# halajun/VDO_SLAM

Measured on AMD Instinct MI355X. Metric: frames/sec (per-frame hot path, KITTI-0000-shaped 1242x375) + ms/LM-iter (batch factor graph), higher is better.
Workload: dtype f64 (LM, RANSAC) / u8,i32,f32 (front-end, tracking)

## Files before the change

include/vdo_slam_hip.h:

```cpp
#ifndef VDO_SLAM_HIP_H_
#define VDO_SLAM_HIP_H_
#include <stdint.h>

#ifdef __cplusplus
extern "C" {
#endif

typedef enum vdo_status {
  VDO_OK = 0,
  VDO_ERR_INVALID = -1,
  VDO_ERR_NO_DEVICE = -2,
  VDO_ERR_OOM = -3,
  VDO_ERR_UNSUPPORTED = -4,
  VDO_ERR_INTERNAL = -5
} vdo_status;

int vdo_version(void);
const char* vdo_last_error(void);

typedef struct vdo_ctx vdo_ctx;
int vdo_ctx_create(int device, void* hip_stream, vdo_ctx** out);
int vdo_ctx_destroy(vdo_ctx* ctx);
int vdo_ctx_synchronize(vdo_ctx* ctx);
int vdo_ctx_stream(vdo_ctx* ctx, void** hip_stream_out);
// ... 74 lines not shown
int vdo_rccl_comm_destroy(vdo_rccl_comm* comm);
int vdo_rccl_comm_stats(const vdo_rccl_comm* comm, int64_t* calls, int64_t* bytes);
int vdo_rccl_allreduce(vdo_rccl_comm* comm, double* device_buf, int64_t count, int op );
int vdo_ba_set_rccl(vdo_ba* ba, vdo_rccl_comm* comm );
int vdo_ba_partition(const vdo_ba_graph* g, int world, int32_t* owner_of_point );
typedef struct vdo_ba_plan vdo_ba_plan;
int vdo_ba_plan_create(const vdo_ba_graph* g, vdo_ba_plan** out);
int vdo_ba_plan_array(const vdo_ba_plan* p, const char* name, const void** data, int64_t* count, int32_t* elem_bytes);
int vdo_ba_plan_destroy(vdo_ba_plan* p);

typedef struct vdo_flow2_problem {
  int32_t n;
  const double* obs;
  const double* flow;
  const double* depth;
  double K[4];
  double Twl[16];
  double T0[16];
  double info_flow;
  double info_prior;
  double huber_delta;
  double chi2_gate;
  int32_t max_iterations;
  int32_t ref_quirks;
} vdo_flow2_problem;

typedef struct vdo_flow2_result {
  double T[16];
  int32_t n_inliers;
  int32_t iterations, trials, stop_reason;
  double initial_chi2, final_chi2, final_lambda;
} vdo_flow2_result;

typedef struct vdo_flow2_batch vdo_flow2_batch;
int vdo_flow2_batch_create(vdo_ctx* ctx, int n_problems, const vdo_flow2_problem* probs, vdo_flow2_batch** out);
int vdo_flow2_batch_reserve(vdo_ctx* ctx, int n_problems, const int32_t* capacity, vdo_flow2_batch** out);
int vdo_flow2_batch_set(vdo_flow2_batch* batch, int k, const vdo_flow2_problem* problem);
int vdo_flow2_batch_run(vdo_flow2_batch* batch);
int vdo_flow2_batch_fetch(vdo_flow2_batch* batch, vdo_flow2_result* results, double** flow_out, uint8_t** inlier_out);
int vdo_flow2_batch_destroy(vdo_flow2_batch* batch);
int vdo_flow2_optimize(vdo_ctx* ctx, const vdo_flow2_problem* p, vdo_flow2_result* result, double* flow_out, uint8_t* inlier_out);

typedef struct vdo_pose_problem {
  int32_t n;
  int32_t kind;
  const double* obs;
  const double* Xw;
  double K[4];
  double P[12];
  double T0[16];
  double huber_delta;
  double chi2_gate;
  int32_t max_iterations;
  int32_t pad;
} vdo_pose_problem;

typedef struct vdo_pose_batch vdo_pose_batch;
int vdo_pose_batch_create(vdo_ctx* ctx, int n_problems, const vdo_pose_problem* probs, vdo_pose_batch** out);
int vdo_pose_batch_run(vdo_pose_batch* batch);
int vdo_pose_batch_fetch(vdo_pose_batch* batch, vdo_flow2_result* results, uint8_t** inlier_out);
int vdo_pose_batch_destroy(vdo_pose_batch* batch);
int vdo_pose_optimize(vdo_ctx* ctx, const vdo_pose_problem* p, vdo_flow2_result* result, uint8_t* inlier_out);

typedef struct vdo_pnp_problem {
  int32_t n;
  const double* X;
  const double* uv;
  double K[4];
  int32_t max_iterations;
  double reproj_threshold;
  double confidence;
  int32_t refit;
} vdo_pnp_problem;
typedef struct vdo_pnp_result {
  double T[16];
  int32_t n_inliers;
  int32_t iterations_run;
  int32_t best_iteration;
} vdo_pnp_result;
int vdo_pnp_ransac_batch(vdo_ctx* ctx, int n_problems, const vdo_pnp_problem* probs, vdo_pnp_result* results, uint8_t** inlier_out);
int vdo_pnp_ransac_batch_overlap(vdo_ctx* ctx, int n_problems, const vdo_pnp_problem* probs, vdo_pnp_result* results, uint8_t** inlier_out,
                                 void (*host_work)(void*), void* host_arg);
int vdo_pnp_ransac(vdo_ctx* ctx, const vdo_pnp_problem* p, vdo_pnp_result* result, uint8_t* inlier_out);

typedef struct vdo_orb_params {
  int32_t n_features;
  float scale_factor;
  int32_t n_levels;
  int32_t ini_th;
  int32_t min_th;
} vdo_orb_params;

typedef struct vdo_keypoints {
  int32_t capacity, n;
  float *x, *y, *response, *angle, *size;
  int32_t* octave;
} vdo_keypoints;

typedef struct vdo_orb vdo_orb;
int vdo_orb_create(vdo_ctx* ctx, const vdo_orb_params* prm, int width, int height, vdo_orb** out);
int vdo_orb_destroy(vdo_orb* orb);
int vdo_orb_max_keypoints(const vdo_orb* orb, int* n);
int vdo_orb_extract(vdo_orb* orb, const uint8_t* gray, int stride, int src_is_device, vdo_keypoints* out);
int vdo_orb_extract_begin(vdo_orb* orb, const uint8_t* gray, int stride, int src_is_device);
int vdo_orb_extract_end(vdo_orb* orb, vdo_keypoints* out);
int vdo_orb_descriptors(vdo_orb* orb, uint8_t* desc32, int capacity_rows);
int vdo_orb_extract_desc(vdo_orb* orb, const uint8_t* gray, int stride, int src_is_device, vdo_keypoints* out, uint8_t* desc32);
int vdo_orb_level_info(vdo_orb* orb, int level, int* w, int* h, int* n_features, int* n_candidates);
int vdo_orb_get_pyramid(vdo_orb* orb, int level, uint8_t* out_bordered );
int vdo_orb_get_blurred(vdo_orb* orb, int level, uint8_t* out );
int vdo_orb_get_candidates(vdo_orb* orb, int level, float* x, float* y, float* response, float* angle, int cap, int* n);
int vdo_orb_last_timing(vdo_orb* orb, double ms[2]);
int vdo_orb_pyramid_launches(const vdo_orb* orb);

int vdo_depth_preprocess(vdo_ctx* ctx, float* depth, int64_t n, float bf, float depth_map_factor, int is_device);
int vdo_rgb2gray(vdo_ctx* ctx, const uint8_t* rgb, int64_t n_pixels, int channels, int rgb_order, uint8_t* gray);

typedef struct vdo_frame_images vdo_frame_images;
int vdo_frame_images_create(vdo_ctx* ctx, int width, int height, vdo_frame_images** out);
int vdo_frame_images_upload(vdo_frame_images* f, const float* depth, const float* flow, const int32_t* mask);
int vdo_frame_images_upload_on(vdo_ctx* ctx, vdo_frame_images* f, const float* depth, const float* flow, const int32_t* mask);
int vdo_frame_images_upload_device(vdo_frame_images* f, const float* depth_dev, const float* flow_dev, const int32_t* mask_dev);
int vdo_frame_images_depth_preprocess(vdo_frame_images* f, float bf, float depth_map_factor);
int vdo_frame_images_ingest_device(vdo_frame_images* f, const float* depth_dev, const float* flow_dev, const int32_t* mask_dev, float bf, float depth_map_factor,
                                   int convert_depth);
int vdo_frame_images_destroy(vdo_frame_images* f);
int vdo_frame_images_set_ctx(vdo_frame_images* f, vdo_ctx* ctx);
int vdo_frame_static_filter(vdo_frame_images* f, int n, const float* kx, const float* ky, float th_depth,
                            int32_t* keep_idx, float* corr_x, float* corr_y, float* flow_x, float* flow_y,
                            float* depth_out, int* n_out);
int vdo_frame_static_filter_sampled(vdo_frame_images* f, int n, const float* kx, const float* ky, float th_depth,
                                    int32_t* keep_idx, float* corr_x, float* corr_y, float* flow_x, float* flow_y,
                                    float* depth_out, int* n_out);
int vdo_sample_keypoints(int rows, int cols, uint64_t seed, int capacity, float* x_out, float* y_out, int* n_out);
int vdo_frame_object_sample(vdo_frame_images* f, float th_depth_obj, int step, int cap,
                            float* key_x, float* key_y, float* corr_x, float* corr_y,
                            float* flow_x, float* flow_y, float* depth_out, int32_t* label, int* n_out);
int vdo_frame_object_sample_on(vdo_ctx* on_ctx, vdo_frame_images* f, float th_depth_obj, int step, int cap,
                               float* key_x, float* key_y, float* corr_x, float* corr_y,
                               float* flow_x, float* flow_y, float* depth_out, int32_t* label, int* n_out);
int vdo_frame_filters(vdo_frame_images* f, int n, const float* kx, const float* ky, float th_depth, int sampled,
                      int32_t* keep_idx, float* s_corr_x, float* s_corr_y, float* s_flow_x, float* s_flow_y, float* s_depth, int* n_static,
                      float th_depth_obj, int step, int cap,
                      float* key_x, float* key_y, float* corr_x, float* corr_y, float* flow_x, float* flow_y, float* depth_out, int32_t* label, int* n_obj);
int vdo_frame_filters_on(vdo_ctx* on_ctx, vdo_frame_images* f, int n, const float* kx, const float* ky, float th_depth, int sampled,
                         int32_t* keep_idx, float* s_corr_x, float* s_corr_y, float* s_flow_x, float* s_flow_y, float* s_depth, int* n_static,
                         float th_depth_obj, int step, int cap,
                         float* key_x, float* key_y, float* corr_x, float* corr_y, float* flow_x, float* flow_y, float* depth_out, int32_t* label, int* n_obj);


int vdo_propagate_static(vdo_frame_images* f, int n, const float* kx, const float* ky, float* depth_out);
int vdo_propagate_object(vdo_frame_images* f, int n, const float* kx, const float* ky, float th_depth_obj,
                         float* depth_out, int32_t* label_out);
int vdo_get3d_world(vdo_ctx* ctx, int n, const float* kx, const float* ky, const float* depth,
                    const float K4[4], const float Twc[16], float* xyz_out);
int vdo_scene_flow(vdo_ctx* ctx, int n, const float* cur_x, const float* cur_y, const float* cur_d, const int32_t* cur_label, const float Tcw_cur[16],
                   const float* last_x, const float* last_y, const float* last_d, const int32_t* last_label, const float Tcw_last[16],
                   const float K4[4], float* flow3d_out, int32_t* obj_label_inout);
int vdo_renew_static(vdo_frame_images* f, int n_tm, const int32_t* tm_sta, const float* stat_x, const float* stat_y,
                     int n_orb, const float* orb_x, const float* orb_y, int max_num_sta,
                     float* key_x, float* key_y, float* corr_x, float* corr_y, float* flow_x, float* flow_y,
                     int32_t* inlier_id, float* depth_out, int* n_out);
int vdo_renew_static_world(vdo_frame_images* f, int n_tm, const int32_t* tm_sta, const float* stat_x, const float* stat_y,
                           int n_orb, const float* orb_x, const float* orb_y, int max_num_sta, const float K4[4], const float Twc[16],
                           float* key_x, float* key_y, float* corr_x, float* corr_y, float* flow_x, float* flow_y,
                           int32_t* inlier_id, float* depth_out, float* xyz_out, int* n_out);
// ... 72 lines not shown
```

vdo_slam_amd/csrc/arena.hpp:

```cpp
#pragma once
#include <hip/hip_runtime.h>

#include <algorithm>
#include <cstdlib>
#include <cstring>
#include <vector>

#include "../../include/vdo_slam_hip.h"
#include "ctx.hpp"

namespace vdo {

class Arena {
 public:
  explicit Arena(vdo_ctx* c) : c_(c), s_(c->stream) {}
  hipStream_t stream() { flush(); return s_; }

  bool reserve(size_t bytes) {
    bytes = (bytes + 4095) & ~size_t(4095);
    if (bytes > c_->d_cap) {
      hipStreamSynchronize(s_);
      if (c_->d_arena) hipFree(c_->d_arena);
      c_->d_arena = nullptr; c_->d_cap = 0;
      const size_t want = bytes < (size_t(8) << 20) ? (size_t(8) << 20) : bytes * 2;
      if (hipMalloc((void**)&c_->d_arena, want) != hipSuccess) return false;
      c_->d_cap = want;
    }
    if (bytes > c_->h_cap) {
      hipStreamSynchronize(s_);
      if (c_->h_arena) hipHostFree(c_->h_arena);
      c_->h_arena = nullptr; c_->h_cap = 0; c_->h_arena_dev = nullptr;
      const size_t want = bytes < (size_t(8) << 20) ? (size_t(8) << 20) : bytes * 2;
      if (hipHostMalloc((void**)&c_->h_arena, want, hipHostMallocMapped) != hipSuccess) return false;
      void* dp = nullptr;
      if (hipHostGetDevicePointer(&dp, c_->h_arena, 0) == hipSuccess) c_->h_arena_dev = (char*)dp;
      c_->h_cap = want;
    }
    off_ = 0; in_lo_ = in_hi_ = 0;
    return true;
  }
  static size_t bytes_for(size_t n_elems_total) { return n_elems_total * 8 + 64 * 256 + 4096; }

  template <class T>
  T* up(const T* host, size_t n) {
    const size_t a = (off_ + 255) & ~size_t(255), bytes = n * sizeof(T);
    if (!c_->d_arena || !c_->h_arena || a + bytes > c_->d_cap || a + bytes > c_->h_cap) return nullptr;
    off_ = a + bytes;
    if (host && n) {
      std::memcpy(c_->h_arena + a, host, bytes);
      if (in_hi_ == in_lo_) { in_lo_ = a; in_hi_ = a + bytes; }
      else if (a - in_hi_ <= 4096) in_hi_ = a + bytes;
      else { flush(); in_lo_ = a; in_hi_ = a + bytes; }
    } else if (in_hi_ != in_lo_ && bytes > 4096) {
      flush();
    }
    return (T*)(c_->d_arena + a);
  }
  template <class T>
  T* out(size_t n) {
    static const bool off = std::getenv("VDO_ARENA_NO_MAPPED_OUT") != nullptr;
    if (off || !c_->h_arena_dev) return up<T>(nullptr, n);
    const size_t a = (off_ + 255) & ~size_t(255), bytes = n * sizeof(T);
    if (!c_->d_arena || !c_->h_arena || a + bytes > c_->d_cap || a + bytes > c_->h_cap) return nullptr;
    off_ = a + bytes;
    if (in_hi_ != in_lo_) flush();
    return (T*)(c_->h_arena_dev + a);
  }
  template <class T>
  void down(T* user, const T* dev, size_t n) {
    if (!user || !n) return;
    if (c_->h_arena_dev && (const char*)dev >= c_->h_arena_dev && (const char*)dev + n * sizeof(T) <= c_->h_arena_dev + c_->h_cap) {
      pend_.push_back({user, (size_t)((const char*)dev - c_->h_arena_dev), n * sizeof(T), true});
      return;
    }
    const size_t o = (size_t)((const char*)dev - c_->d_arena);
    if ((const char*)dev < c_->d_arena || o + n * sizeof(T) > c_->d_cap) { failed_ = true; return; }
    pend_.push_back({user, o, n * sizeof(T), false});
  }
  template <class T>
  const T* down_view(const T* dev, size_t n) {
    const size_t o = (size_t)((const char*)dev - c_->d_arena);
    if ((const char*)dev < c_->d_arena || o + n * sizeof(T) > c_->d_cap) { failed_ = true; return nullptr; }
    if (n) pend_.push_back({nullptr, o, n * sizeof(T), false});
    return (const T*)(c_->h_arena + o);
  }
  void queue_downloads() {
    if (queued_) return;
    queued_ = true;
    flush();
    {
      size_t lo = ~size_t(0), hi = 0, sum = 0;
      for (const Pend& p : pend_) if (!p.mapped) { lo = std::min(lo, p.off); hi = std::max(hi, p.off + p.bytes); sum += p.bytes; }
      if (sum) {
        bool overlap = false;
        for (const Pend& p : pend_) if (p.mapped && p.off < hi && p.off + p.bytes > lo) overlap = true;
        if (!overlap && hi - lo <= 4 * sum + (size_t(64) << 10)) hipMemcpyAsync(c_->h_arena + lo, c_->d_arena + lo, hi - lo, hipMemcpyDeviceToHost, s_);
        else for (const Pend& p : pend_) if (!p.mapped) hipMemcpyAsync(c_->h_arena + p.off, c_->d_arena + p.off, p.bytes, hipMemcpyDeviceToHost, s_);
      }
    }
  }
  int finish(const char* what) {
    queue_downloads();
    queued_ = false;
    hipError_t e = hipStreamSynchronize(s_);
    if (e == hipSuccess) e = hipGetLastError();
    if (e != hipSuccess) { pend_.clear(); return set_error(VDO_ERR_NO_DEVICE, "%s: %s", what, hipGetErrorString(e)); }
    if (failed_) { pend_.clear(); return set_error(VDO_ERR_OOM, "%s: scratch arena exhausted", what); }
    for (const Pend& p : pend_) if (p.user) std::memcpy(p.user, c_->h_arena + p.off, p.bytes);
    pend_.clear();
    return VDO_OK;
  }

 private:
  void flush() {
    if (in_hi_ != in_lo_) hipMemcpyAsync(c_->d_arena + in_lo_, c_->h_arena + in_lo_, in_hi_ - in_lo_, hipMemcpyHostToDevice, s_);
    in_lo_ = in_hi_ = 0;
  }
  struct Pend { void* user; size_t off, bytes; bool mapped; };
  vdo_ctx* c_;
  hipStream_t s_;
  size_t off_ = 0, in_lo_ = 0, in_hi_ = 0;
  bool failed_ = false, queued_ = false;
  std::vector<Pend> pend_;
};

}
```

vdo_slam_amd/csrc/ransac.hip:

```cpp
#include <algorithm>
#include <cfloat>
#include <chrono>
#include <cmath>
#include <cstdlib>
#include <cstring>
#include <mutex>
#include <unordered_map>
#include <vector>

#include "../../include/vdo_slam_hip.h"
#include "arena.hpp"
#include "ctx.hpp"
#include "epnp_refit.hpp"
#include "host_pool.hpp"

namespace vdo {

struct PnpDev {
  int n, n_hyp, pt_off, hyp_off, mask_off, mask_words, pad0, pad1;
  double K[4];
  double thr2;
};

__device__ __forceinline__ double d3dot(const double* a, const double* b) { return a[0] * b[0] + a[1] * b[1] + a[2] * b[2]; }
__device__ __forceinline__ void d3cross(const double* a, const double* b, double* o) { o[0] = a[1] * b[2] - a[2] * b[1]; o[1] = a[2] * b[0] - a[0] * b[2]; o[2] = a[0] * b[1] - a[1] * b[0]; }
__device__ __forceinline__ bool d3unit(double* a) { const double n = sqrt(d3dot(a, a)); if (!(n > 1e-300)) return false; a[0] /= n; a[1] /= n; a[2] /= n; return true; }

__device__ __forceinline__ double cbrt_exact(double x) {
  if (x == 0 || x != x) return x;
  unsigned long long bits = (unsigned long long)__double_as_longlong(x);
  const unsigned long long sign = bits & 0x8000000000000000ULL;
  bits &= 0x7fffffffffffffffULL;
  int bexp = (int)(bits >> 52), adj = 0;
  if (bexp == 0x7ff) return x;
  if (bexp == 0) {
    bits = (unsigned long long)__double_as_longlong(__longlong_as_double((long long)bits) * 18014398509481984.0);
    bexp = (int)(bits >> 52); adj = -18;
  }
  const int e = bexp - 1023;
  const int k = (e >= 0 ? e : e - 2) / 3, r = e - 3 * k;
  const unsigned long long frac = bits & 0x000fffffffffffffULL;
  const double f = __longlong_as_double((long long)(frac | (1023ULL << 52)));
  const double m = __longlong_as_double((long long)(frac | ((unsigned long long)(1023 + r) << 52)));
  double y = (1.0 + (f - 1.0) * 0.26) * (r == 0 ? 1.0 : r == 1 ? 1.2599210498948732 : 1.5874010519681994);
#pragma unroll
  for (int it = 0; it < 6; ++it) y = y - (y * y * y - m) / (3.0 * (y * y));
  const double s = __longlong_as_double((long long)((unsigned long long)(1023 + k + adj) << 52));
  return __longlong_as_double((long long)((unsigned long long)__double_as_longlong(y * s) | sign));
}

__device__ __forceinline__ double cubic3_largest_root(double P, double Q) {
  double t = 2 * sqrt(-P / 3);
  for (int it = 0; it < 64; ++it) {
    const double f = (t * t + P) * t + Q, fp = 3 * (t * t) + P;
    if (!(fp > 0)) break;
    const double tn = t - f / fp;
    if (!(tn < t)) break;
    t = tn;
  }
  return t;
}

__device__ int quartic_real_roots(double b, double c, double d, double e, double* roots) {
  const double p = c - 3 * b * b / 8, q = d - b * c / 2 + b * b * b / 8, r = e - b * d / 4 + b * b * c / 16 - 3 * b * b * b * b / 256;
  double y[4];
  int n = 0;
  const double scale = fabs(p) + fabs(r) + 1e-300;
  if (fabs(q) < 1e-14 * scale) {
    const double disc = p * p - 4 * r;
    if (disc >= 0) {
      const double s = sqrt(disc);
      const double w0 = (-p + s) / 2, w1 = (-p - s) / 2;
      if (w0 >= 0) { y[n++] = sqrt(w0); y[n++] = -sqrt(w0); }
      if (w1 >= 0) { y[n++] = sqrt(w1); y[n++] = -sqrt(w1); }
    }
  } else {
    const double A = 2 * p, B = p * p - 4 * r, C = -q * q;
    const double P = B - A * A / 3, Q = 2 * A * A * A / 27 - A * B / 3 + C;
    const double disc = Q * Q / 4 + P * P * P / 27;
    double t;
    if (disc >= 0) {
      const double s = sqrt(disc);
      t = cbrt_exact(-Q / 2 + s) + cbrt_exact(-Q / 2 - s);
    } else {
      t = cubic3_largest_root(P, Q);
    }
    double z = t - A / 3;
#pragma unroll
    for (int it = 0; it < 3; ++it) {
      const double f = ((z + A) * z + B) * z + C, fp = (3 * z + 2 * A) * z + B;
      if (fp != 0) z -= f / fp;
    }
    if (z > 0) {
      const double s = sqrt(z);
      const double h1 = (p + z - q / s) / 2, h2 = (p + z + q / s) / 2;
      const double d1 = s * s - 4 * h1, d2 = s * s - 4 * h2;
      if (d1 >= 0) { const double w = sqrt(d1); y[n++] = (-s + w) / 2; y[n++] = (-s - w) / 2; }
      if (d2 >= 0) { const double w = sqrt(d2); y[n++] = (s + w) / 2; y[n++] = (s - w) / 2; }
    }
  }
  for (int i = 0; i < n; ++i) {
    double x = y[i] - b / 4;
// ... 218 lines not shown
      if (!(fabs(ct1) <= 1)) continue;
      double st1 = sqrt(1 - ct1 * ct1);
      st1 = (k3b3 > 0) ? st1 : -st1;
      double ct3 = g1 * ct1 + g2, st3 = g3 * ct1 + g4;
      const double nt3 = st1 / ((g5 * ct1 + g6) * ct1 + g7);
      ct3 *= nt3; st3 *= nt3;
      const double C13[9] = {ct3, 0, -st3, st1 * st3, ct1, st1 * ct3, ct1 * st3, -st1, ct1 * ct3};
      double tm[9], Rw[9];
#pragma unroll
      for (int a = 0; a < 3; ++a)
#pragma unroll
        for (int b = 0; b < 3; ++b) tm[3 * a + b] = Ck[3 * a] * C13[b] + Ck[3 * a + 1] * C13[3 + b] + Ck[3 * a + 2] * C13[6 + b];
#pragma unroll
      for (int a = 0; a < 3; ++a)
#pragma unroll
        for (int b = 0; b < 3; ++b) Rw[3 * a + b] = tm[3 * a] * Cb[b] + tm[3 * a + 1] * Cb[3 + b] + tm[3 * a + 2] * Cb[6 + b];
      const double rp3[3] = {w3[0] * Rw[0] + w3[1] * Rw[3] + w3[2] * Rw[6], w3[0] * Rw[1] + w3[1] * Rw[4] + w3[2] * Rw[7], w3[0] * Rw[2] + w3[1] * Rw[5] + w3[2] * Rw[8]};
      double R[9], t[3];
      bool fin = true;
#pragma unroll
      for (int a = 0; a < 3; ++a) {
        t[a] = st1 * b3p[a] - rp3[a];
        fin = fin && d_finite(t[a]);
#pragma unroll
        for (int b = 0; b < 3; ++b) { R[3 * a + b] = Rw[3 * b + a]; fin = fin && d_finite(R[3 * a + b]); }
      }
      if (!fin) continue;
      const double e4 = reproj_err2(R, t, P.K, P4, u4, v4);
      if (!ok || best > e4) {
        best = e4; ok = 1;
#pragma unroll
        for (int q = 0; q < 9; ++q) out[q] = R[q];
        out[9] = t[0]; out[10] = t[1]; out[11] = t[2];
      }
    }
  } while (false);
  if (ok) {
    double R[9];
#pragma unroll
    for (int q = 0; q < 9; ++q) R[q] = out[q];
    polar_orthogonalise(R);
#pragma unroll
    for (int q = 0; q < 9; ++q) { out[q] = R[q]; ok = ok && d_finite(R[q]); }
  }
  hyp_ok[P.hyp_off + h] = ok;
}

__global__ __launch_bounds__(256) void k_ransac_vote(const PnpDev* __restrict__ probs, const double* __restrict__ X, const double* __restrict__ uv,
                                                     const double* __restrict__ hyp_pose, const int32_t* __restrict__ hyp_ok,
                                                     int32_t* __restrict__ count, uint32_t* __restrict__ mask) {
  const PnpDev P = probs[blockIdx.y];
  const int h = blockIdx.x;
  if (h >= P.n_hyp) return;
  __shared__ int s_cnt[4];
  const int gh = P.hyp_off + h;
  uint32_t* mrow = mask + (size_t)P.mask_off + (size_t)h * P.mask_words;
  if (!hyp_ok[gh]) {
    for (int w = threadIdx.x; w < P.mask_words; w += 256) mrow[w] = 0;
    if (threadIdx.x == 0) count[gh] = 0;
    return;
  }
  double R[9], t[3];
#pragma unroll
  for (int i = 0; i < 9; ++i) R[i] = hyp_pose[12 * (size_t)gh + i];
  t[0] = hyp_pose[12 * (size_t)gh + 9]; t[1] = hyp_pose[12 * (size_t)gh + 10]; t[2] = hyp_pose[12 * (size_t)gh + 11];
  const double* Xp = X + 3 * (size_t)P.pt_off;
  const double* up = uv + 2 * (size_t)P.pt_off;
  int c = 0;
  const int n_pad = (P.n + 63) & ~63;
  for (int i = threadIdx.x; i < n_pad; i += 256) {
    bool in = false;
    if (i < P.n) in = reproj_err2(R, t, P.K, Xp + 3 * i, up[2 * i], up[2 * i + 1]) <= P.thr2;
    const unsigned long long b = __ballot(in);
    c += in;
    if ((threadIdx.x & 63) == 0) { mrow[i >> 5] = (uint32_t)b; if ((i >> 5) + 1 < P.mask_words) mrow[(i >> 5) + 1] = (uint32_t)(b >> 32); }
  }
#pragma unroll
  for (int off = 32; off > 0; off >>= 1) c += __shfl_down(c, off, 64);
  if ((threadIdx.x & 63) == 0) s_cnt[threadIdx.x >> 6] = c;
  __syncthreads();
  if (threadIdx.x == 0) count[gh] = s_cnt[0] + s_cnt[1] + s_cnt[2] + s_cnt[3];
}

struct CvRng {
  uint64_t state;
  explicit CvRng(uint64_t s) : state(s ? s : 0xffffffffULL) {}
  unsigned next() { state = (uint64_t)(unsigned)state * 4164903690U + (unsigned)(state >> 32); return (unsigned)state; }
  int uniform(int a, int b) { return a == b ? a : (int)(next() % (unsigned)(b - a) + a); }
};

static int ransac_update_iters(double p, double ep, int model_points, int max_iters) {
  p = std::min(1.0, std::max(0.0, p)); ep = std::min(1.0, std::max(0.0, ep));
  double num = std::max(1.0 - p, DBL_MIN);
  double denom = 1.0 - std::pow(1.0 - ep, model_points);
  if (denom < DBL_MIN) return 0;
  num = std::log(num); denom = std::log(denom);
  return denom >= 0 || -num >= max_iters * (-denom) ? max_iters : (int)std::lrint(num / denom);
}

}

using namespace vdo;

namespace {
struct PnpTrace {
  std::mutex mu;
  double t[5] = {0, 0, 0, 0, 0}; long n = 0; bool on = std::getenv("VDO_PNP_TRACE") != nullptr;
  ~PnpTrace() { if (on && n) std::fprintf(stderr, "[pnp trace] calls %ld: setup %.1f us, gpu %.1f us, replay %.1f us, refit %.1f us (per call)\n", n, t[0] / n, t[1] / n, t[2] / n, t[3] / n); }
} g_pnp_trace;
inline double pnp_now_us() { return std::chrono::duration<double, std::micro>(std::chrono::steady_clock::now().time_since_epoch()).count(); }
}

extern "C" int vdo_pnp_ransac_batch_overlap(vdo_ctx* ctx, int n_problems, const vdo_pnp_problem* probs, vdo_pnp_result* results, uint8_t** inlier_out,
                                            void (*host_work)(void*), void* host_arg) {
  if (!ctx || !probs || !results || n_problems <= 0) return set_error(VDO_ERR_INVALID, "vdo_pnp_ransac_batch: bad argument");
  const double tr0 = g_pnp_trace.on ? pnp_now_us() : 0.0;
  int rc = ctx_bind(ctx);
  if (rc != VDO_OK) return rc;
  static thread_local std::vector<PnpDev> hp;
  static thread_local std::vector<int32_t> subsets;
  static thread_local std::vector<double> X, uv;
  hp.assign(n_problems, PnpDev{});
  size_t tot_pts = 0, tot_hyp = 0, tot_words = 0;
  int max_hyp = 0;
  for (int k = 0; k < n_problems; ++k) {
    const vdo_pnp_problem& p = probs[k];
    if (p.n < 0 || p.max_iterations < 0 || (p.n > 0 && (!p.X || !p.uv))) return set_error(VDO_ERR_INVALID, "pnp problem %d: bad fields", k);
    PnpDev& d = hp[k];
    d.n = p.n; d.n_hyp = p.n >= 4 ? p.max_iterations : 0;
    d.pt_off = (int)tot_pts; d.hyp_off = (int)tot_hyp; d.mask_off = (int)tot_words; d.mask_words = (p.n + 63) / 64 * 2;
    std::memcpy(d.K, p.K, sizeof d.K);
    d.thr2 = p.reproj_threshold * p.reproj_threshold;
    tot_pts += p.n; tot_hyp += d.n_hyp; tot_words += (size_t)d.n_hyp * d.mask_words;
    max_hyp = std::max(max_hyp, d.n_hyp);
  }
  for (int k = 0; k < n_problems; ++k) {
    vdo_pnp_result& r = results[k];
    for (int i = 0; i < 16; ++i) r.T[i] = (i % 5 == 0) ? 1.0 : 0.0;
    r.n_inliers = 0; r.iterations_run = 0; r.best_iteration = -1;
    if (inlier_out && inlier_out[k] && probs[k].n) std::memset(inlier_out[k], 0, (size_t)probs[k].n);
  }
  if (tot_hyp == 0) { if (host_work) host_work(host_arg); return VDO_OK; }
  subsets.resize(4 * tot_hyp);
  X.resize(3 * tot_pts); uv.resize(2 * tot_pts);
  {
    static std::mutex cache_mu;
    static std::unordered_map<uint64_t, std::vector<int32_t>> cache;
    for (int k = 0; k < n_problems; ++k) {
      const PnpDev& d = hp[k];
      if (d.n) { std::memcpy(X.data() + 3 * (size_t)d.pt_off, probs[k].X, sizeof(double) * 3 * d.n); std::memcpy(uv.data() + 2 * (size_t)d.pt_off, probs[k].uv, sizeof(double) * 2 * d.n); }
      if (!d.n_hyp) continue;
      int32_t* dst = subsets.data() + 4 * (size_t)d.hyp_off;
      const uint64_t key = ((uint64_t)(uint32_t)d.n << 32) | (uint32_t)d.n_hyp;
      {
        std::lock_guard<std::mutex> g(cache_mu);
        auto it = cache.find(key);
        if (it != cache.end()) { std::memcpy(dst, it->second.data(), sizeof(int32_t) * 4 * (size_t)d.n_hyp); continue; }
      }
      CvRng rng((uint64_t)-1);
      for (int it = 0; it < d.n_hyp; ++it) {
        int32_t* s = dst + 4 * (size_t)it;
        for (int i = 0; i < 4; ++i)
          for (;;) {
            const int c = rng.uniform(0, d.n);
            bool dup = false;
            for (int j = 0; j < i; ++j) dup |= (s[j] == c);
            if (!dup) { s[i] = c; break; }
          }
      }
      std::lock_guard<std::mutex> g(cache_mu);
      if (cache.size() < 4096) cache.emplace(key, std::vector<int32_t>(dst, dst + 4 * (size_t)d.n_hyp));
    }
  }
  const double tr1 = g_pnp_trace.on ? pnp_now_us() : 0.0;
  Arena S(ctx);
  if (!S.reserve(40 * tot_pts + 128 * tot_hyp + 4 * tot_words + sizeof(PnpDev) * (size_t)n_problems + 16 * 256 + 8192))
    return set_error(VDO_ERR_OOM, "scratch arena: allocation failed");
  PnpDev* dprob = S.up(hp.data(), (size_t)n_problems);
  double *dX = S.up(X.data(), X.size()), *duv = S.up(uv.data(), uv.size());
  int32_t* dsub = S.up(subsets.data(), subsets.size());
  double* dpose = S.up<double>(nullptr, 12 * tot_hyp);
  int32_t *dok = S.up<int32_t>(nullptr, tot_hyp), *dcnt = S.up<int32_t>(nullptr, tot_hyp);
  uint32_t* dmask = S.up<uint32_t>(nullptr, tot_words);
  if (!dprob || !dX || !duv || !dsub || !dpose || !dok || !dcnt || !dmask) return set_error(VDO_ERR_OOM, "scratch arena exhausted");
  bool grunert = true;
  for (int k = 0; k < n_problems; ++k) grunert = grunert && (probs[k].refit & 2);
  for (int k = 0; k < n_problems; ++k) if (((probs[k].refit & 2) != 0) != grunert) return set_error(VDO_ERR_INVALID, "vdo_pnp_ransac_batch: the problems of a batch must name the same minimal solver");
  if (grunert) hipLaunchKernelGGL(k_p3p_hyp, dim3((max_hyp + 63) / 64, n_problems), dim3(64), 0, S.stream(), (const PnpDev*)dprob, (const double*)dX, (const double*)duv, (const int32_t*)dsub, dpose, dok);
  else hipLaunchKernelGGL(k_ap3p_hyp, dim3((max_hyp + 63) / 64, n_problems), dim3(64), 0, S.stream(), (const PnpDev*)dprob, (const double*)dX, (const double*)duv, (const int32_t*)dsub, dpose, dok);
  hipLaunchKernelGGL(k_ransac_vote, dim3(max_hyp, n_problems), dim3(256), 0, S.stream(), (const PnpDev*)dprob, (const double*)dX, (const double*)duv, (const double*)dpose, (const int32_t*)dok, dcnt, dmask);
  const int32_t *cnt = S.down_view(dcnt, tot_hyp), *okv = S.down_view(dok, tot_hyp);
  const double* pose = S.down_view(dpose, 12 * tot_hyp);
  const uint32_t* mask = S.down_view(dmask, tot_words);
  S.queue_downloads();
  if (host_work) host_work(host_arg);
  rc = S.finish("vdo_pnp_ransac_batch");
  if (rc != VDO_OK) return rc;
  if (!cnt || !okv || !pose || !mask) return set_error(VDO_ERR_OOM, "scratch arena exhausted");
  const double tr2 = g_pnp_trace.on ? pnp_now_us() : 0.0;
  for (int k = 0; k < n_problems; ++k) {
    const PnpDev& d = hp[k];
    if (!d.n_hyp) continue;
    int niters = d.n_hyp, max_good = 0, it = 0, bi = -1;
    for (; it < niters; ++it) {
      const int g = d.hyp_off + it;
      if (!okv[g]) continue;
      if (cnt[g] > std::max(max_good, 3)) {
        max_good = cnt[g]; bi = it;
        niters = ransac_update_iters(probs[k].confidence, (double)(d.n - cnt[g]) / d.n, 4, niters);
      }
    }
    vdo_pnp_result& r = results[k];
    r.iterations_run = it; r.best_iteration = bi; r.n_inliers = max_good;
    if (bi < 0) continue;
    const double* Pz = pose + 12 * ((size_t)d.hyp_off + bi);
    for (int i = 0; i < 3; ++i) { for (int j = 0; j < 3; ++j) r.T[4 * i + j] = Pz[3 * i + j]; r.T[4 * i + 3] = Pz[9 + i]; }
    if (inlier_out && inlier_out[k]) {
      const uint32_t* row = mask + (size_t)d.mask_off + (size_t)bi * d.mask_words;
      for (int i = 0; i < d.n; ++i) inlier_out[k][i] = (row[i >> 5] >> (i & 31)) & 1u;
    }
  }
  const double tr3 = g_pnp_trace.on ? pnp_now_us() : 0.0;
  std::vector<int> todo;
  for (int k = 0; k < n_problems; ++k) if ((probs[k].refit & 1) && results[k].n_inliers >= 4 && results[k].best_iteration >= 0) todo.push_back(k);
  if (!todo.empty()) {
    const PnpDev* hp_main = hp.data();
    auto refit_one = [&, hp_main](int q) {
      const int k = todo[q];
      const PnpDev& d = hp_main[k];
      const uint32_t* row = mask + (size_t)d.mask_off + (size_t)results[k].best_iteration * d.mask_words;
      thread_local std::vector<double> Xi, ui;
      thread_local epnp::Scratch scr;
      Xi.clear(); ui.clear();
      for (int i = 0; i < d.n; ++i)
        if ((row[i >> 5] >> (i & 31)) & 1u) {
          Xi.insert(Xi.end(), probs[k].X + 3 * (size_t)i, probs[k].X + 3 * (size_t)i + 3);
          ui.insert(ui.end(), probs[k].uv + 2 * (size_t)i, probs[k].uv + 2 * (size_t)i + 2);
        }
      const epnp::Result r = epnp::solve((int)(ui.size() / 2), Xi.data(), ui.data(), probs[k].K, scr);
      if (r.err >= 0.0)
        for (int i = 0; i < 3; ++i) { for (int j = 0; j < 3; ++j) results[k].T[4 * i + j] = r.R[3 * i + j]; results[k].T[4 * i + 3] = r.t[i]; }
    };
    static LevelPool* pool = [] {
      const char* e = std::getenv("VDO_PNP_THREADS");
      const int nw = e ? std::atoi(e) : 3;
      return nw > 0 ? new LevelPool(std::min(nw, 15)) : nullptr;
    }();
    static std::mutex pool_mu;
    if (todo.size() > 1 && pool && pool_mu.try_lock()) {
      pool->run((int)todo.size(), refit_one);
      pool_mu.unlock();
    } else {
      for (int q = 0; q < (int)todo.size(); ++q) refit_one(q);
    }
  }
  if (g_pnp_trace.on && n_problems > 1) {
    const double tr4 = pnp_now_us();
    std::lock_guard<std::mutex> lock(g_pnp_trace.mu);
    g_pnp_trace.t[0] += tr1 - tr0; g_pnp_trace.t[1] += tr2 - tr1; g_pnp_trace.t[2] += tr3 - tr2; g_pnp_trace.t[3] += tr4 - tr3; ++g_pnp_trace.n;
  }
  return VDO_OK;
}

extern "C" int vdo_pnp_ransac_batch(vdo_ctx* ctx, int n_problems, const vdo_pnp_problem* probs, vdo_pnp_result* results, uint8_t** inlier_out) {
  return vdo_pnp_ransac_batch_overlap(ctx, n_problems, probs, results, inlier_out, nullptr, nullptr);
}
extern "C" int vdo_pnp_ransac(vdo_ctx* ctx, const vdo_pnp_problem* p, vdo_pnp_result* result, uint8_t* inlier_out) {
  return vdo_pnp_ransac_batch(ctx, 1, p, result, &inlier_out);
}
```

vdo_slam_amd/ransac.py:

```python
import ctypes as C

import numpy as np

from . import _capi as K


class PnpProblemC(C.Structure):
    _fields_ = [("n", C.c_int32), ("X", K.c_double_p), ("uv", K.c_double_p), ("K", C.c_double * 4),
                ("max_iterations", C.c_int32), ("reproj_threshold", C.c_double), ("confidence", C.c_double), ("refit", C.c_int32)]


class PnpResultC(C.Structure):
    _fields_ = [("T", C.c_double * 16), ("n_inliers", C.c_int32), ("iterations_run", C.c_int32), ("best_iteration", C.c_int32)]


def pnp_ransac_batch(ctx, problems, K4, max_iterations=500, thr=0.4, confidence=0.98, refit=False, solver="ap3p"):
    flags = int(bool(refit)) | (2 if solver == "grunert" else 0)
    n = len(problems)
    arr = (PnpProblemC * n)()
    keep, inl = [], []
    for i, (X, uv) in enumerate(problems):
        X = np.ascontiguousarray(X, dtype=np.float64).reshape(-1, 3); uv = np.ascontiguousarray(uv, dtype=np.float64).reshape(-1, 2)
        keep += [X, uv]
        arr[i] = PnpProblemC(X.shape[0], K._dp(X), K._dp(uv), (C.c_double * 4)(*K4), max_iterations, thr, confidence, flags)
        inl.append(np.zeros(max(X.shape[0], 1), np.uint8))
    res = (PnpResultC * n)()
    ip = (K.c_uint8_p * n)(*[a.ctypes.data_as(K.c_uint8_p) for a in inl])
    L = K.lib()
    L.vdo_pnp_ransac_batch.argtypes = [C.c_void_p, C.c_int, C.POINTER(PnpProblemC), C.POINTER(PnpResultC), C.POINTER(K.c_uint8_p)]
    K.check(L.vdo_pnp_ransac_batch(ctx._h, n, arr, res, ip))
    return [dict(T=np.array(res[i].T).reshape(4, 4), n_inliers=res[i].n_inliers, iterations_run=res[i].iterations_run,
                 best_iteration=res[i].best_iteration, inliers=inl[i][:keep[2 * i].shape[0]]) for i in range(n)]
```

Measured before the change: 1349.

## Compact RANSAC best-so-far records on GPU to shrink device-to-host readback

```diff
diff --git a/include/vdo_slam_hip.h b/include/vdo_slam_hip.h
--- a/include/vdo_slam_hip.h
+++ b/include/vdo_slam_hip.h
@@ -180,6 +180,7 @@
 int vdo_pnp_ransac_batch_overlap(vdo_ctx* ctx, int n_problems, const vdo_pnp_problem* probs, vdo_pnp_result* results, uint8_t** inlier_out,
                                  void (*host_work)(void*), void* host_arg);
 int vdo_pnp_ransac(vdo_ctx* ctx, const vdo_pnp_problem* p, vdo_pnp_result* result, uint8_t* inlier_out);
+void vdo_pnp_path_counts(int64_t out[4]);
 
 typedef struct vdo_orb_params {
   int32_t n_features;
diff --git a/vdo_slam_amd/csrc/arena.hpp b/vdo_slam_amd/csrc/arena.hpp
--- a/vdo_slam_amd/csrc/arena.hpp
+++ b/vdo_slam_amd/csrc/arena.hpp
@@ -57,6 +57,20 @@
     return (T*)(c_->d_arena + a);
   }
   template <class T>
+  T* up_fill(size_t n, T** host_slot) {
+    const size_t a = (off_ + 255) & ~size_t(255), bytes = n * sizeof(T);
+    *host_slot = nullptr;
+    if (!c_->d_arena || !c_->h_arena || a + bytes > c_->d_cap || a + bytes > c_->h_cap) return nullptr;
+    off_ = a + bytes;
+    *host_slot = (T*)(c_->h_arena + a);
+    if (n) {
+      if (in_hi_ == in_lo_) { in_lo_ = a; in_hi_ = a + bytes; }
+      else if (a - in_hi_ <= 4096) in_hi_ = a + bytes;
+      else { flush(); in_lo_ = a; in_hi_ = a + bytes; }
+    }
+    return (T*)(c_->d_arena + a);
+  }
+  template <class T>
   T* out(size_t n) {
     static const bool off = std::getenv("VDO_ARENA_NO_MAPPED_OUT") != nullptr;
     if (off || !c_->h_arena_dev) return up<T>(nullptr, n);
@@ -83,6 +97,12 @@
     if ((const char*)dev < c_->d_arena || o + n * sizeof(T) > c_->d_cap) { failed_ = true; return nullptr; }
     if (n) pend_.push_back({nullptr, o, n * sizeof(T), false});
     return (const T*)(c_->h_arena + o);
+  }
+  template <class T>
+  const T* out_view(const T* dev, size_t n) {
+    if (c_->h_arena_dev && (const char*)dev >= c_->h_arena_dev && (const char*)dev + n * sizeof(T) <= c_->h_arena_dev + c_->h_cap)
+      return (const T*)(c_->h_arena + ((const char*)dev - c_->h_arena_dev));
+    return down_view(dev, n);
   }
   void queue_downloads() {
     if (queued_) return;
diff --git a/vdo_slam_amd/csrc/ransac.hip b/vdo_slam_amd/csrc/ransac.hip
--- a/vdo_slam_amd/csrc/ransac.hip
+++ b/vdo_slam_amd/csrc/ransac.hip
@@ -1,4 +1,5 @@
 #include <algorithm>
+#include <atomic>
 #include <cfloat>
 #include <chrono>
 #include <cmath>
@@ -17,7 +18,7 @@
 namespace vdo {
 
 struct PnpDev {
-  int n, n_hyp, pt_off, hyp_off, mask_off, mask_words, pad0, pad1;
+  int n, n_hyp, pt_off, hyp_off, mask_off, mask_words, rec_off, pad1;
   double K[4];
   double thr2;
 };
@@ -402,6 +403,45 @@
   if (threadIdx.x == 0) count[gh] = s_cnt[0] + s_cnt[1] + s_cnt[2] + s_cnt[3];
 }
 
+__global__ __launch_bounds__(64) void k_ransac_records(const PnpDev* __restrict__ probs, const int32_t* __restrict__ hyp_ok, const int32_t* __restrict__ count,
+                                                       const double* __restrict__ hyp_pose, const uint32_t* __restrict__ mask, int cap,
+                                                       int32_t* __restrict__ rec_n, int32_t* __restrict__ rec_it, double* __restrict__ rec_pose,
+                                                       uint32_t* __restrict__ rec_mask) {
+  const PnpDev P = probs[blockIdx.x];
+  const int lane = threadIdx.x;
+  int run_max = 3, nrec = 0;
+  for (int base = 0; base < P.n_hyp; base += 64) {
+    const int it = base + lane;
+    int v = 0;
+    if (it < P.n_hyp && hyp_ok[P.hyp_off + it]) v = count[P.hyp_off + it];
+    int inc = v;
+#pragma unroll
+    for (int off = 1; off < 64; off <<= 1) { const int o = __shfl_up(inc, off, 64); if (lane >= off) inc = max(inc, o); }
+    int before = __shfl_up(inc, 1, 64);
+    if (lane == 0) before = 0;
+    unsigned long long todo = __ballot(v > max(run_max, before));
+    while (todo) {
+      const int src = __ffsll((long long)todo) - 1;
+      todo &= todo - 1;
+      const int cnt = __shfl(v, src, 64);
+      if (nrec < cap) {
+        const int h = base + src;
+        const size_t slot = (size_t)blockIdx.x * cap + nrec;
+        if (lane == 0) { rec_it[2 * slot] = h; rec_it[2 * slot + 1] = cnt; }
+        if (lane < 12) rec_pose[12 * slot + lane] = hyp_pose[12 * (size_t)(P.hyp_off + h) + lane];
+        const uint32_t* row = mask + (size_t)P.mask_off + (size_t)h * P.mask_words;
+        uint32_t* dst = rec_mask + (size_t)P.rec_off + (size_t)nrec * P.mask_words;
+        for (int w = lane; w < P.mask_words; w += 64) dst[w] = row[w];
+      }
+      ++nrec;
+    }
+    run_max = max(run_max, __shfl(inc, 63, 64));
+  }
+  if (lane == 0) rec_n[blockIdx.x] = nrec;
+}
+
+constexpr int kPnpRecordCap = 32;
+
 struct CvRng {
   uint64_t state;
   explicit CvRng(uint64_t s) : state(s ? s : 0xffffffffULL) {}
@@ -425,10 +465,22 @@
 namespace {
 struct PnpTrace {
   std::mutex mu;
-  double t[5] = {0, 0, 0, 0, 0}; long n = 0; bool on = std::getenv("VDO_PNP_TRACE") != nullptr;
-  ~PnpTrace() { if (on && n) std::fprintf(stderr, "[pnp trace] calls %ld: setup %.1f us, gpu %.1f us, replay %.1f us, refit %.1f us (per call)\n", n, t[0] / n, t[1] / n, t[2] / n, t[3] / n); }
+  double t[2][4] = {{0, 0, 0, 0}, {0, 0, 0, 0}}; long n[2] = {0, 0};
+  double bytes[2] = {0, 0};
+  long fallbacks = 0, full_copies = 0; int max_records = 0;
+  bool on = std::getenv("VDO_PNP_TRACE") != nullptr;
+  ~PnpTrace() {
+    if (!on) return;
+    static const char* const what[2] = {"", " (one problem)"};
+    for (int q = 0; q < 2; ++q)
+      if (n[q]) std::fprintf(stderr, "[pnp trace%s] calls %ld: setup %.1f us, gpu %.1f us, replay %.1f us, refit %.1f us (per call); %.0f bytes to the host per call\n", what[q], n[q],
+                             t[q][0] / n[q], t[q][1] / n[q], t[q][2] / n[q], t[q][3] / n[q], bytes[q] / n[q]);
+    if (n[0] + n[1]) std::fprintf(stderr, "[pnp trace] records per problem: at most %d; calls that fell back to the full arrays: %ld; calls with VDO_PNP_FULL_COPY: %ld\n", max_records, fallbacks, full_copies);
+  }
 } g_pnp_trace;
 inline double pnp_now_us() { return std::chrono::duration<double, std::micro>(std::chrono::steady_clock::now().time_since_epoch()).count(); }
+std::atomic<int64_t> g_pnp_paths[4];
+inline bool env_on(const char* name) { const char* e = std::getenv(name); return e && *e && std::strcmp(e, "0") != 0; }
 }
 
 extern "C" int vdo_pnp_ransac_batch_overlap(vdo_ctx* ctx, int n_problems, const vdo_pnp_problem* probs, vdo_pnp_result* results, uint8_t** inlier_out,
@@ -437,21 +489,25 @@
   const double tr0 = g_pnp_trace.on ? pnp_now_us() : 0.0;
   int rc = ctx_bind(ctx);
   if (rc != VDO_OK) return rc;
+  bool full = env_on("VDO_PNP_FULL_COPY");
+  int cap = kPnpRecordCap;
+  if (const char* e = std::getenv("VDO_PNP_RECORD_CAP")) cap = std::min(kPnpRecordCap, std::max(1, std::atoi(e)));
   static thread_local std::vector<PnpDev> hp;
-  static thread_local std::vector<int32_t> subsets;
-  static thread_local std::vector<double> X, uv;
+  static thread_local std::vector<const double*> best_pose;
+  static thread_local std::vector<const uint32_t*> best_row;
   hp.assign(n_problems, PnpDev{});
-  size_t tot_pts = 0, tot_hyp = 0, tot_words = 0;
+  best_pose.assign(n_problems, nullptr); best_row.assign(n_problems, nullptr);
+  size_t tot_pts = 0, tot_hyp = 0, tot_words = 0, tot_rec_words = 0;
   int max_hyp = 0;
   for (int k = 0; k < n_problems; ++k) {
     const vdo_pnp_problem& p = probs[k];
     if (p.n < 0 || p.max_iterations < 0 || (p.n > 0 && (!p.X || !p.uv))) return set_error(VDO_ERR_INVALID, "pnp problem %d: bad fields", k);
     PnpDev& d = hp[k];
     d.n = p.n; d.n_hyp = p.n >= 4 ? p.max_iterations : 0;
-    d.pt_off = (int)tot_pts; d.hyp_off = (int)tot_hyp; d.mask_off = (int)tot_words; d.mask_words = (p.n + 63) / 64 * 2;
+    d.pt_off = (int)tot_pts; d.hyp_off = (int)tot_hyp; d.mask_off = (int)tot_words; d.mask_words = (p.n + 63) / 64 * 2; d.rec_off = (int)tot_rec_words;
     std::memcpy(d.K, p.K, sizeof d.K);
     d.thr2 = p.reproj_threshold * p.reproj_threshold;
-    tot_pts += p.n; tot_hyp += d.n_hyp; tot_words += (size_t)d.n_hyp * d.mask_words;
+    tot_pts += p.n; tot_hyp += d.n_hyp; tot_words += (size_t)d.n_hyp * d.mask_words; tot_rec_words += (size_t)cap * d.mask_words;
     max_hyp = std::max(max_hyp, d.n_hyp);
   }
   for (int k = 0; k < n_problems; ++k) {
@@ -461,16 +517,26 @@
     if (inlier_out && inlier_out[k] && probs[k].n) std::memset(inlier_out[k], 0, (size_t)probs[k].n);
   }
   if (tot_hyp == 0) { if (host_work) host_work(host_arg); return VDO_OK; }
-  subsets.resize(4 * tot_hyp);
-  X.resize(3 * tot_pts); uv.resize(2 * tot_pts);
+  Arena S(ctx);
+  if (!S.reserve(40 * tot_pts + 128 * tot_hyp + 4 * tot_words + sizeof(PnpDev) * (size_t)n_problems + 16 * 256 + 8192 +
+                 (size_t)n_problems * (4 + (size_t)cap * (8 + 96)) + 4 * tot_rec_words + 4 * 256))
+    return set_error(VDO_ERR_OOM, "scratch arena: allocation failed");
+  PnpDev* dprob = S.up(hp.data(), (size_t)n_problems);
+  double *hX = nullptr, *huv = nullptr;
+  double* dX = S.up_fill<double>(3 * tot_pts, &hX);
+  if (dX) for (int k = 0; k < n_problems; ++k) if (hp[k].n) std::memcpy(hX + 3 * (size_t)hp[k].pt_off, probs[k].X, sizeof(double) * 3 * hp[k].n);
+  double* duv = S.up_fill<double>(2 * tot_pts, &huv);
+  if (duv) for (int k = 0; k < n_problems; ++k) if (hp[k].n) std::memcpy(huv + 2 * (size_t)hp[k].pt_off, probs[k].uv, sizeof(double) * 2 * hp[k].n);
+  int32_t* hsub = nullptr;
+  int32_t* dsub = S.up_fill<int32_t>(4 * tot_hyp, &hsub);
+  if (!dprob || !dX || !duv || !dsub) return set_error(VDO_ERR_OOM, "scratch arena exhausted");
   {
     static std::mutex cache_mu;
     static std::unordered_map<uint64_t, std::vector<int32_t>> cache;
     for (int k = 0; k < n_problems; ++k) {
       const PnpDev& d = hp[k];
-      if (d.n) { std::memcpy(X.data() + 3 * (size_t)d.pt_off, probs[k].X, sizeof(double) * 3 * d.n); std::memcpy(uv.data() + 2 * (size_t)d.pt_off, probs[k].uv, sizeof(double) * 2 * d.n); }
       if (!d.n_hyp) continue;
-      int32_t* dst = subsets.data() + 4 * (size_t)d.hyp_off;
+      int32_t* dst = hsub + 4 * (size_t)d.hyp_off;
       const uint64_t key = ((uint64_t)(uint32_t)d.n << 32) | (uint32_t)d.n_hyp;
       {
         std::lock_guard<std::mutex> g(cache_mu);
@@ -493,50 +559,93 @@
     }
   }
   const double tr1 = g_pnp_trace.on ? pnp_now_us() : 0.0;
-  Arena S(ctx);
-  if (!S.reserve(40 * tot_pts + 128 * tot_hyp + 4 * tot_words + sizeof(PnpDev) * (size_t)n_problems + 16 * 256 + 8192))
-    return set_error(VDO_ERR_OOM, "scratch arena: allocation failed");
-  PnpDev* dprob = S.up(hp.data(), (size_t)n_problems);
-  double *dX = S.up(X.data(), X.size()), *duv = S.up(uv.data(), uv.size());
-  int32_t* dsub = S.up(subsets.data(), subsets.size());
   double* dpose = S.up<double>(nullptr, 12 * tot_hyp);
   int32_t *dok = S.up<int32_t>(nullptr, tot_hyp), *dcnt = S.up<int32_t>(nullptr, tot_hyp);
   uint32_t* dmask = S.up<uint32_t>(nullptr, tot_words);
-  if (!dprob || !dX || !duv || !dsub || !dpose || !dok || !dcnt || !dmask) return set_error(VDO_ERR_OOM, "scratch arena exhausted");
+  if (!dpose || !dok || !dcnt || !dmask) return set_error(VDO_ERR_OOM, "scratch arena exhausted");
   bool grunert = true;
   for (int k = 0; k < n_problems; ++k) grunert = grunert && (probs[k].refit & 2);
   for (int k = 0; k < n_problems; ++k) if (((probs[k].refit & 2) != 0) != grunert) return set_error(VDO_ERR_INVALID, "vdo_pnp_ransac_batch: the problems of a batch must name the same minimal solver");
   if (grunert) hipLaunchKernelGGL(k_p3p_hyp, dim3((max_hyp + 63) / 64, n_problems), dim3(64), 0, S.stream(), (const PnpDev*)dprob, (const double*)dX, (const double*)duv, (const int32_t*)dsub, dpose, dok);
   else hipLaunchKernelGGL(k_ap3p_hyp, dim3((max_hyp + 63) / 64, n_problems), dim3(64), 0, S.stream(), (const PnpDev*)dprob, (const double*)dX, (const double*)duv, (const int32_t*)dsub, dpose, dok);
   hipLaunchKernelGGL(k_ransac_vote, dim3(max_hyp, n_problems), dim3(256), 0, S.stream(), (const PnpDev*)dprob, (const double*)dX, (const double*)duv, (const double*)dpose, (const int32_t*)dok, dcnt, dmask);
-  const int32_t *cnt = S.down_view(dcnt, tot_hyp), *okv = S.down_view(dok, tot_hyp);
-  const double* pose = S.down_view(dpose, 12 * tot_hyp);
-  const uint32_t* mask = S.down_view(dmask, tot_words);
+  const int32_t *cnt = nullptr, *okv = nullptr, *rec_n = nullptr, *rec_it = nullptr;
+  const double *pose = nullptr, *rec_pose = nullptr;
+  const uint32_t *mask = nullptr, *rec_mask = nullptr;
+  auto view_all = [&] {
+    cnt = S.down_view(dcnt, tot_hyp); okv = S.down_view(dok, tot_hyp);
+    pose = S.down_view(dpose, 12 * tot_hyp);
+    mask = S.down_view(dmask, tot_words);
+  };
+  if (full) view_all();
+  else {
+    int32_t *orn = S.out<int32_t>((size_t)n_problems), *orit = S.out<int32_t>(2 * (size_t)cap * n_problems);
+    double* orpose = S.out<double>(12 * (size_t)cap * n_problems);
+    uint32_t* ormask = S.out<uint32_t>(tot_rec_words);
+    if (!orn || !orit || !orpose || !ormask) return set_error(VDO_ERR_OOM, "scratch arena exhausted");
+    hipLaunchKernelGGL(k_ransac_records, dim3(n_problems), dim3(64), 0, S.stream(), (const PnpDev*)dprob, (const int32_t*)dok, (const int32_t*)dcnt, (const double*)dpose,
+                       (const uint32_t*)dmask, cap, orn, orit, orpose, ormask);
+    rec_n = S.out_view(orn, (size_t)n_problems); rec_it = S.out_view(orit, 2 * (size_t)cap * n_problems);
+    rec_pose = S.out_view(orpose, 12 * (size_t)cap * n_problems); rec_mask = S.out_view(ormask, tot_rec_words);
+  }
   S.queue_downloads();
   if (host_work) host_work(host_arg);
   rc = S.finish("vdo_pnp_ransac_batch");
   if (rc != VDO_OK) return rc;
-  if (!cnt || !okv || !pose || !mask) return set_error(VDO_ERR_OOM, "scratch arena exhausted");
+  double bytes_back = 0.0;
+  int max_rec = 0;
+  bool fell_back = false;
+  if (!full) {
+    if (!rec_n || !rec_it || !rec_pose || !rec_mask) return set_error(VDO_ERR_OOM, "scratch arena exhausted");
+    for (int k = 0; k < n_problems; ++k) {
+      max_rec = std::max(max_rec, rec_n[k]);
+      bytes_back += 4.0 + (double)std::min(rec_n[k], cap) * (8 + 96 + 4 * hp[k].mask_words);
+    }
+    if (max_rec > cap) {
+      fell_back = full = true;
+      view_all();
+      rc = S.finish("vdo_pnp_ransac_batch");
+      if (rc != VDO_OK) return rc;
+    }
+  }
+  if (full) {
+    if (!cnt || !okv || !pose || !mask) return set_error(VDO_ERR_OOM, "scratch arena exhausted");
+    bytes_back += 104.0 * tot_hyp + 4.0 * tot_words;
+  }
+  g_pnp_paths[fell_back ? 1 : full ? 2 : 0].fetch_add(1, std::memory_order_relaxed);
+  for (int64_t seen = g_pnp_paths[3].load(std::memory_order_relaxed); seen < max_rec && !g_pnp_paths[3].compare_exchange_weak(seen, max_rec, std::memory_order_relaxed);) {}
   const double tr2 = g_pnp_trace.on ? pnp_now_us() : 0.0;
   for (int k = 0; k < n_problems; ++k) {
     const PnpDev& d = hp[k];
     if (!d.n_hyp) continue;
     int niters = d.n_hyp, max_good = 0, it = 0, bi = -1;
-    for (; it < niters; ++it) {
-      const int g = d.hyp_off + it;
-      if (!okv[g]) continue;
-      if (cnt[g] > std::max(max_good, 3)) {
-        max_good = cnt[g]; bi = it;
-        niters = ransac_update_iters(probs[k].confidence, (double)(d.n - cnt[g]) / d.n, 4, niters);
+    if (full) {
+      for (; it < niters; ++it) {
+        const int g = d.hyp_off + it;
+        if (!okv[g]) continue;
+        if (cnt[g] > std::max(max_good, 3)) {
+          max_good = cnt[g]; bi = it;
+          niters = ransac_update_iters(probs[k].confidence, (double)(d.n - cnt[g]) / d.n, 4, niters);
+        }
       }
+      if (bi >= 0) { best_pose[k] = pose + 12 * ((size_t)d.hyp_off + bi); best_row[k] = mask + (size_t)d.mask_off + (size_t)bi * d.mask_words; }
+    } else {
+      const int32_t* ri = rec_it + 2 * (size_t)k * cap;
+      for (int r = 0; r < rec_n[k]; ++r) {
+        if (ri[2 * r] >= niters) break;
+        bi = ri[2 * r]; max_good = ri[2 * r + 1];
+        niters = ransac_update_iters(probs[k].confidence, (double)(d.n - max_good) / d.n, 4, niters);
+        best_pose[k] = rec_pose + 12 * ((size_t)k * cap + r); best_row[k] = rec_mask + (size_t)d.rec_off + (size_t)r * d.mask_words;
+      }
+      it = bi >= 0 ? std::max(niters, bi + 1) : niters;
     }
     vdo_pnp_result& r = results[k];
     r.iterations_run = it; r.best_iteration = bi; r.n_inliers = max_good;
     if (bi < 0) continue;
-    const double* Pz = pose + 12 * ((size_t)d.hyp_off + bi);
+    const double* Pz = best_pose[k];
     for (int i = 0; i < 3; ++i) { for (int j = 0; j < 3; ++j) r.T[4 * i + j] = Pz[3 * i + j]; r.T[4 * i + 3] = Pz[9 + i]; }
     if (inlier_out && inlier_out[k]) {
-      const uint32_t* row = mask + (size_t)d.mask_off + (size_t)bi * d.mask_words;
+      const uint32_t* row = best_row[k];
       for (int i = 0; i < d.n; ++i) inlier_out[k][i] = (row[i >> 5] >> (i & 31)) & 1u;
     }
   }
@@ -545,10 +654,11 @@
   for (int k = 0; k < n_problems; ++k) if ((probs[k].refit & 1) && results[k].n_inliers >= 4 && results[k].best_iteration >= 0) todo.push_back(k);
   if (!todo.empty()) {
     const PnpDev* hp_main = hp.data();
-    auto refit_one = [&, hp_main](int q) {
+    const uint32_t* const* row_main = best_row.data();
+    auto refit_one = [&, hp_main, row_main](int q) {
       const int k = todo[q];
       const PnpDev& d = hp_main[k];
-      const uint32_t* row = mask + (size_t)d.mask_off + (size_t)results[k].best_iteration * d.mask_words;
+      const uint32_t* row = row_main[k];
       thread_local std::vector<double> Xi, ui;
       thread_local epnp::Scratch scr;
       Xi.clear(); ui.clear();
@@ -574,14 +684,20 @@
       for (int q = 0; q < (int)todo.size(); ++q) refit_one(q);
     }
   }
-  if (g_pnp_trace.on && n_problems > 1) {
+  if (g_pnp_trace.on) {
     const double tr4 = pnp_now_us();
+    const int q = n_problems > 1 ? 0 : 1;
     std::lock_guard<std::mutex> lock(g_pnp_trace.mu);
-    g_pnp_trace.t[0] += tr1 - tr0; g_pnp_trace.t[1] += tr2 - tr1; g_pnp_trace.t[2] += tr3 - tr2; g_pnp_trace.t[3] += tr4 - tr3; ++g_pnp_trace.n;
+    g_pnp_trace.t[q][0] += tr1 - tr0; g_pnp_trace.t[q][1] += tr2 - tr1; g_pnp_trace.t[q][2] += tr3 - tr2; g_pnp_trace.t[q][3] += tr4 - tr3; ++g_pnp_trace.n[q];
+    g_pnp_trace.bytes[q] += bytes_back; g_pnp_trace.max_records = std::max(g_pnp_trace.max_records, max_rec);
+    g_pnp_trace.fallbacks += fell_back; g_pnp_trace.full_copies += (full && !fell_back);
   }
   return VDO_OK;
 }
 
+extern "C" void vdo_pnp_path_counts(int64_t out[4]) {
+  if (out) for (int i = 0; i < 4; ++i) out[i] = g_pnp_paths[i].load(std::memory_order_relaxed);
+}
 extern "C" int vdo_pnp_ransac_batch(vdo_ctx* ctx, int n_problems, const vdo_pnp_problem* probs, vdo_pnp_result* results, uint8_t** inlier_out) {
   return vdo_pnp_ransac_batch_overlap(ctx, n_problems, probs, results, inlier_out, nullptr, nullptr);
 }
diff --git a/vdo_slam_amd/ransac.py b/vdo_slam_amd/ransac.py
--- a/vdo_slam_amd/ransac.py
+++ b/vdo_slam_amd/ransac.py
@@ -31,3 +31,12 @@
     K.check(L.vdo_pnp_ransac_batch(ctx._h, n, arr, res, ip))
     return [dict(T=np.array(res[i].T).reshape(4, 4), n_inliers=res[i].n_inliers, iterations_run=res[i].iterations_run,
                  best_iteration=res[i].best_iteration, inliers=inl[i][:keep[2 * i].shape[0]]) for i in range(n)]
+
+
+def pnp_path_counts():
+    out = (C.c_int64 * 4)()
+    L = K.lib()
+    L.vdo_pnp_path_counts.argtypes = [C.POINTER(C.c_int64)]
+    L.vdo_pnp_path_counts.restype = None
+    L.vdo_pnp_path_counts(out)
+    return tuple(int(v) for v in out)
```

After: 1327. 0.984x the previous value.
